# SamsungLabs/Metis

Hardware: NVIDIA H100
Metric: candidate plans evaluated/sec (higher is better)
Workload: dtype f64

## Files before the change

### metis_b200/csrc/metis_coop.cuh

```cuda
#pragma once

#include "metis_eval.cuh"

namespace metis {

struct CoopMail {
    int m;
    int err;
    int flag;
    int aux;
    double val;
    double val2;
    int k;
    int s_top;
    int top_skip;
    int pad2;
};

struct OneLane {
    bool reverse = false;
    MB_HD int lane() const { return 0; }
    MB_HD int width() const { return 1; }
    MB_HD bool leader() const { return true; }
    MB_HD void sync() const {}
    MB_HD bool any(bool p) const { return p; }
    MB_HD unsigned ballot(bool p) const { return p ? 1u : 0u; }
    MB_HD unsigned match_any(int) const { return 1u; }
    MB_HD int first_ge_window(const double *P, int n, int i0, int lo, double t) const {
        for (int k = 0; k < 32 && i0 + k <= n; ++k)
            if (P[i0 + k] >= t) return (k > 0 || i0 <= lo) ? i0 + k : -1;
        return -1;
    }
    MB_HD int first_ge(const double *P, int n, double t) const {
        int lo = 0, hi = n + 1;
        while (lo < hi) { const int mid = (lo + hi) >> 1; if (P[mid] >= t) hi = mid; else lo = mid + 1; }
        return lo;
    }
    MB_HD int bcast_last(int v) const { return v; }
    MB_HD static void assume_shared(const void *) {}
    MB_HD void argmax_first(double &, int &) const {}
    MB_HD void argmin_first(double &, int &) const {}
    MB_HD void imax_first(int &, int &) const {}
    MB_HD void imin_first(int &, int &) const {}
    MB_HD double max_all(double v) const { return v; }
    MB_HD int incl_scan(int v) const { return v; }
    MB_HD int last_lane(int v) const { return v; }
    MB_HD void mark(int) const {}
    MB_HD void note(int) const {}
    MB_HD void gate(int, int) const {}
};

enum CoopGate { kGateRun = 0, kGateBackward = 1, kGateLeftover = 2, kGateVote = 3, kGateAdjust = 4, kGateMemory = 5,
                kGateCost = 6 };

template <class X>
MB_HD int par_index(const X &, int i, int n) { (void)n; return i; }
MB_HD int par_index(const OneLane &x, int i, int n) { return x.reverse ? n - 1 - i : i; }

#define METIS_PAR(x, var, n) \
    for (int var##_i = (x).lane(), var = par_index((x), var##_i, (n)); var##_i < (n); \
         var##_i += (x).width(), var = par_index((x), var##_i, (n)))

struct FillState {
    int k;
    int s_top;
    bool top_skip;
};

template <int MAXS, int MAXL>
MB_HD_NOINLINE FillState seq_forward(const Tables &T, int S, Scratch<MAXS, MAXL> &w) {
    const int L = T.p.num_layers;
    const double *dlay = T.dlay;
    const int N = kH * L;
    const int lim = (N - 1 - kH) > 0 ? (N - 1 - kH) : 0;
    const int last = S - 1;
    FillState st{0, -1, false};
    if (S > 1) {
        int s = 0, j = 0;
        double c = w.capa[0];
        bool done = false;
#pragma unroll 1
        for (int r = 0; r + 1 < L && !done; ++r) {
            const double d = dlay[r];
            const int nsub = (r == L - 2) ? kH - 1 : kH;
            if (nsub == kH && c > 9.0 * d) {
                c -= d; c -= d; c -= d; c -= d; c -= d; c -= d; c -= d;
                j += kH;
                continue;
            }
#pragma unroll
            for (int q = 0; q < kH; ++q) {
                if (q < nsub && !done) {
                    if (c > d) {
                        c -= d;
                    } else {
                        w.capa[s] = c;
                        w.fe[s] = (uint16_t)((j + q) | kBroke);
                        ++s;
                        if (s >= last) done = true;
                        else c = w.capa[s];
                    }
                }
            }
            j += nsub;
        }
        if (s < last) {
            w.capa[s] = c;
            w.fe[s] = (uint16_t)lim;
#pragma unroll 1
            for (int t = s + 1; t < last; ++t) w.fe[t] = (uint16_t)lim;
            st.k = lim;
            st.s_top = s;
        } else {
            st.k = (w.fe[last - 1] & kPos) + 1;
            st.s_top = last - 1;
            st.top_skip = true;
        }
    }
    return st;
}

template <int MAXS, int MAXL>
MB_HD_NOINLINE int seq_backward(const Tables &T, int S, Scratch<MAXS, MAXL> &w, int k) {
    const int L = T.p.num_layers;
    const double *dlay = T.dlay;
    const int N = kH * L;
    const int last = S - 1;
    double c = w.capa[last];
    int r = L - 1;
    double d = dlay[r];
#pragma unroll 1
    for (int i = 0; i < kH; ++i) c -= d;
    int m = N - kH;
    bool full = false;
#pragma unroll 1
    while (m > k && !full) {
        --r;
        d = dlay[r];
        const int floor_j = kH * r > k ? kH * r : k;
#pragma unroll 1
        while (m > floor_j) {
            if (!(c > d)) { full = true; break; }
            c -= d;
            --m;
        }
    }
    if (!full) {
        int sp = S - 2;
#pragma unroll 1
        while (m > 0) {
            const int j = m - 1;
#pragma unroll 1
            while (sp >= 0 && (!(w.fe[sp] & kBroke) || (int)(w.fe[sp] & kPos) > j)) --sp;
            if (!(sp >= 0 && (int)(w.fe[sp] & kPos) == j)) break;
            const double dj = dlay[j / kH];
            if (!(c > dj)) break;
            c -= dj;
            m = j;
            w.fe[sp] |= kTaken;
        }
    }
    w.capa[last] = c;
    return m;
}

template <int MAXS, int MAXL>
MB_HD_NOINLINE int seq_skipped(const Tables &T, int S, Scratch<MAXS, MAXL> &w) {
    const double *dlay = T.dlay;
    const int last = S - 1;
    int start = 0;
#pragma unroll 1
    for (int s = 0; s < last; ++s) {
        const uint16_t e = w.fe[s];
        const int pos = e & kPos;
        const int next_start = pos + ((e & kBroke) ? 1 : 0);
        if ((e & (kBroke | kTaken)) != kBroke) { start = next_start; continue; }
        const int j = pos;
        int lo = 0;
        if (pos > start) {
            lo = s;
        } else {
#pragma unroll 1
            for (int u = s;; --u) {
                if (u < s) {
                    const int t = w.lstk[u];
                    const bool above = (t == last) || (fwd_nonempty(w, t) && fwd_start(w, t) > j);
                    if (!above) { lo = t; break; }
                }
                if (fwd_nonempty(w, u)) { lo = u; break; }
                if (u == 0) break;
            }
        }
        int hi = s + 1;
        if (hi < last && !((int)(w.fe[hi] & kPos) > next_start && !w.got[hi])) {
            ++hi;
#pragma unroll 1
            while (hi < last && (!fwd_nonempty(w, hi) || w.got[hi])) ++hi;
        }
        if (lo > hi) return METIS_FATAL_SCRATCH;
        int pick = lo;
        double best = w.capa[lo];
#pragma unroll 1
        for (int t = lo + 1; t <= hi; ++t)
            if (w.capa[t] > best) { best = w.capa[t]; pick = t; }
        w.capa[pick] -= dlay[j / kH];
        w.lstk[s] = (uint8_t)pick;
        w.got[pick] = 1;
        start = next_start;
    }
    return METIS_FATAL_NONE;
}

template <int MAXS, int MAXL>
MB_HD int middle_lo(int S, const Scratch<MAXS, MAXL> &w, const FillState &st) {
    const int last = S - 1;
    if (st.s_top < 0) return 0;
#pragma unroll 1
    for (int u = st.s_top;; --u) {
        if (u < st.s_top || st.top_skip) {
            const uint16_t eu = w.fe[u];
            if ((eu & (kBroke | kTaken)) == kBroke) {
                const int t2 = w.lstk[u];
                if (t2 != last) return t2;
            }
        }
        if (fwd_nonempty(w, u)) return u;
        if (u == 0) break;
    }
    return 0;
}

MB_HD_NOINLINE double seq_py_sum(const double *v, int n) {
    if (n <= 0) return 0.0;
    double f = 0.0 + v[0], c = 0.0;
#pragma unroll 4
    for (int i = 1; i < n; ++i) {
        const double x = v[i];
        const double t = f + x;
        if (fabs(f) >= fabs(x)) c += (f - t) + x;
        else c += (x - t) + f;
        f = t;
    }
    if (c != 0.0 && isfinite(c)) f += c;
    return f;
}

template <int MAXS, int MAXL, class X, bool ONE = false>
struct CoopEvaluator : PlanEvaluator<MAXS, MAXL, SerialUniform, ONE> {
    using Base = PlanEvaluator<MAXS, MAXL, SerialUniform, ONE>;
    using Base::T; using Base::w; using Base::pd; using Base::bs_total; using Base::nbad; using Base::aux;
    X x;
    CoopMail &mail;

    MB_HD CoopEvaluator(const Tables &t, Scratch<MAXS, MAXL> &s, CoopMail &mb, const X &lanes)
        : Base(t, s), x(lanes), mail(mb) {}

    MB_HD void shared_scratch() const { X::assume_shared(&w); X::assume_shared(&mail); }

    MB_HD void begin_coop(const PlanDesc &plan) {
        shared_scratch();
        pd = plan;
        bs_total = T.p.gbs / pd.batches;
        int lb = 0;
#pragma unroll 1
        while ((2 << lb) <= bs_total) ++lb;
        nbad = 0;
        x.sync();
        int carry = 0;
#pragma unroll 1
        for (int base = 0; base < pd.S; base += x.width()) {
            const int s = base + x.lane();
            const int g = s < pd.S ? pd.row[s] : 0;
            const int sz = s < pd.S ? (1 << g) : 0;
            const int inc = x.incl_scan(sz);
            if (s < pd.S) {
                w.gcode[s] = (uint8_t)g;
                w.tpc[s] = (uint8_t)(g > lb ? g - lb : 0);
                w.rs[s] = (uint16_t)(carry + inc - sz);
            }
            carry += x.last_lane(inc);
        }
        if (x.leader()) w.rs[pd.S] = (uint16_t)carry;
        x.sync();
    }

    MB_HD bool next_strategy_coop(bool have_state) {
        shared_scratch();
        int pick = 0x7FFFFFFF;
        if (have_state) {
            double best = INFINITY;
            bool none = true;
            METIS_PAR(x, s, pd.S) {
                if (w.gcode[s] != w.tpc[s] && (none || w.mstate[s] < best || (w.mstate[s] == best && s < pick))) {
                    pick = s; best = w.mstate[s]; none = false;
                }
            }
            x.argmin_first(best, pick);
        } else {
            int best = -1;
            METIS_PAR(x, s, pd.S) {
                const int ldp = (int)w.gcode[s] - (int)w.tpc[s];
                if (ldp != 0 && (ldp > best || (ldp == best && s < pick))) { pick = s; best = ldp; }
            }
            x.imax_first(best, pick);
        }
        if (pick == 0x7FFFFFFF) return false;
        const int g = w.gcode[pick], t = w.tpc[pick];
        nbad += (this->stage_bad(g, t + 1) ? 1 : 0) - (this->stage_bad(g, t) ? 1 : 0);
        x.sync();
        if (x.leader()) w.tpc[pick] = (uint8_t)(t + 1);
        x.sync();
        return true;
    }

    MB_HD_NOINLINE int first_error(const double *box, int n) {
        shared_scratch();
        x.sync();
        if (x.leader()) {
            mail.err = 0;
#pragma unroll 1
            for (int s = 0; s < n; ++s)
                if (box[s] != 0.0) {
                    uint32_t a;
                    mail.err = decode_error(box[s], a);
                    mail.aux = (int)a;
                    break;
                }
        }
        x.sync();
        aux = (uint32_t)mail.aux;
        return mail.err;
    }

    MB_HD int compute_performance_coop() {
        shared_scratch();
        bool failed = false;
        x.sync();
        METIS_PAR(x, s, pd.S) {
            double p;
            const int rc = this->stage_performance(s, p);
            w.perf[s] = p;
            w.extra[s] = encode_error(rc, aux);
            failed = failed || rc != 0;
        }
        if (x.any(failed)) return first_error(w.extra, pd.S);
        x.sync();
        if (x.leader()) mail.val = seq_py_sum(w.perf, pd.S);
        x.sync();
        const double tot = mail.val;
        if (tot == 0.0) return METIS_FATAL_ZERODIV;
        METIS_PAR(x, s, pd.S) w.perf[s] = w.perf[s] / tot;
        x.sync();
        return 0;
    }

    MB_HD bool forward_coop() {
        shared_scratch();
        const int S = pd.S, last = S - 1;
        const int L = T.p.num_layers;
        if (S < 4 || T.p.norm_len < L) { x.note(kPathSeqForward); return false; }
        const int N = kH * L;
        const int lim = (N - 1 - kH) > 0 ? (N - 1 - kH) : 0;
        const double *dsub = T.dsub;
        const double *P = T.psub;
        int a = 0, first_open = -1;
        int span = lim / last;
#pragma unroll 1
        for (int s = 0; s < last; ++s) {
            int b = lim;
            bool closed = false;
            if (a < lim) {
                const double t = w.perf[s] + P[a];
                int i0 = a + span - 14;
                if (i0 < a + 1) i0 = a + 1;
                int i = x.first_ge_window(P, N, i0, a + 1, t);
                if (i < 0) { x.note(kPathFirstGe); i = x.first_ge(P, N, t); }
                b = i - 1 > a ? i - 1 : a;
                if (b >= lim) b = lim; else closed = true;
                span = b - a;
            }
            if (x.leader()) { w.first[s] = (uint16_t)a; w.fe[s] = (uint16_t)(b | (closed ? kBroke : 0)); }
            if (!closed && first_open < 0) first_open = s;
            a = closed ? b + 1 : lim;
        }
        x.sync();
        x.mark(19);
        bool bad = false;
        METIS_PAR(x, s, last) {
            const int st = w.first[s];
            const uint16_t e = w.fe[s];
            const int b = e & kPos;
            double c = w.perf[s];
            bool fits = true;
#pragma unroll 4
            for (int j = st; j < b; ++j) {
                const double d = dsub[j];
                fits &= c > d;
                c -= d;
            }
            if (!fits || ((e & kBroke) && c > dsub[b])) bad = true;
            w.capa[s] = c;
        }
        if (x.any(bad)) {
            x.note(kPathVerifyFailed);
            x.sync();
            METIS_PAR(x, s, last) w.capa[s] = w.perf[s];
            return false;
        }
        if (x.leader()) {
            if (first_open < 0) { mail.k = a; mail.s_top = last - 1; mail.top_skip = 1; }
            else { mail.k = lim; mail.s_top = first_open; mail.top_skip = 0; }
        }
        return true;
    }

    MB_HD int fill_coop() {
        shared_scratch();
        const int S = pd.S, last = S - 1;
        const double *dlay = T.dlay;
        x.sync();
        const bool fwd = forward_coop();
        x.sync();
        x.gate(kGateBackward, 11);
        if (x.leader()) {
            if (!fwd) {
                x.mark(18);
                const FillState st = seq_forward<MAXS, MAXL>(T, S, w);
                mail.k = st.k; mail.s_top = st.s_top; mail.top_skip = st.top_skip ? 1 : 0;
                x.mark(11);
            }
            mail.m = seq_backward<MAXS, MAXL>(T, S, w, mail.k);
            mail.err = 0;
        }
        x.sync();
        x.gate(kGateLeftover, 12);
        const FillState st{mail.k, mail.s_top, mail.top_skip != 0};
        const int m = mail.m;
        if (st.s_top >= 0 && !st.top_skip) x.note(kPathTail);
        const int reach = st.s_top;
        bool irregular = false;
        METIS_PAR(x, s, reach + 1) {
            const int start = s == 0 ? 0 : (int)(w.fe[s - 1] & kPos) + ((w.fe[s - 1] & kBroke) ? 1 : 0);
            if (!((int)(w.fe[s] & kPos) > start)) irregular = true;
        }
        irregular = x.any(irregular);
        if (irregular) {
            x.note(kPathIrregular);
            if (x.leader()) mail.err = seq_skipped<MAXS, MAXL>(T, S, w);
            x.sync();
            if (mail.err) return mail.err;
        } else if (reach >= 0) {
            int carry = 0;
#pragma unroll 1
            for (int base = 0; base <= last; base += x.width()) {
                const int s = base + x.lane();
                bool has = false, o0 = false, o1 = false, has_prev = false;
                double c = 0.0, d = 0.0, d_prev = 0.0;
                int pos = 0;
                if (s <= last) {
                    c = w.capa[s];
                    if (s > 0 && s - 1 < last) {
                        const uint16_t ep = w.fe[s - 1];
                        has_prev = (ep & (kBroke | kTaken)) == kBroke;
                        if (has_prev) d_prev = dlay[(ep & kPos) / kH];
                    }
                    if (s < last) {
                        const uint16_t e = w.fe[s];
                        has = (e & (kBroke | kTaken)) == kBroke;
                        if (has) {
                            pos = e & kPos;
                            d = dlay[pos / kH];
                            const double cn = w.capa[s + 1];
                            o0 = cn > c;
                            o1 = has_prev ? cn > (c - d_prev) : o0;
                        }
                    }
                }
                const unsigned kmask = x.ballot(o0 == o1), vmask = x.ballot(o0);
                const unsigned below_me = x.lane() ? (0xFFFFFFFFu >> (32 - x.lane())) : 0u;
                const unsigned kin = kmask & below_me;
                const bool in = kin ? ((vmask >> (31 - clz32(kin))) & 1u) != 0u : carry != 0;
                const bool up = (o0 == o1) ? o0 : in;
                carry = x.bcast_last(up ? 1 : 0);
                x.sync();
                if (s <= last) {
                    double cc = c;
                    const bool got_prev = has_prev && in;
                    if (got_prev) cc -= d_prev;
                    if (has && !up) cc -= d;
                    if (got_prev || (has && !up)) w.capa[s] = cc;
                    if (has) w.lstk[s] = (uint8_t)(up ? s + 1 : s);
                }
            }
            x.sync();
        }
        x.mark(17);
        if (m > st.k) {
            x.note(kPathMiddle);
            if (x.leader()) mail.flag = middle_lo<MAXS, MAXL>(S, w, st);
            x.sync();
            int lo = mail.flag;
#pragma unroll 1
            for (int j = st.k; j < m; ++j) {
                int pick = 0x7FFFFFFF;
                double best = -INFINITY;
#pragma unroll 1
                for (int t = lo + x.lane(); t <= last; t += x.width())
                    if (w.capa[t] > best || (w.capa[t] == best && t < pick)) { best = w.capa[t]; pick = t; }
                x.argmax_first(best, pick);
                x.sync();
                if (x.leader()) {
                    w.capa[pick] = best - dlay[j / kH];
                    reinterpret_cast<uint8_t *>(w.subw)[j - st.k] = (uint8_t)pick;
                }
                x.sync();
                if (pick != last) lo = pick;
            }
        }
        return METIS_FATAL_NONE;
    }

    MB_HD int balance_coop() {
        shared_scratch();
        const int S = pd.S;
        const int L = T.p.num_layers;
        if (T.p.norm_len < L) return METIS_FATAL_INDEX;
        const double *lc = T.norm_lc;
        const int last = S - 1;
        x.sync();
        METIS_PAR(x, s, S) { w.capa[s] = w.perf[s]; w.got[s] = 0; }
        x.sync();
        x.mark(10);
        const int rc_tail = fill_coop();
        if (rc_tail) return rc_tail;
        const int m = mail.m;
        x.gate(kGateVote, 13);
        const int kfwd = mail.k;
        const int B = (L + 31) >> 5;
        METIS_PAR(x, blk, 32) {
            const int r0 = blk * B, r1 = r0 + B < L ? r0 + B : L;
            const int j0 = kH * r0;
            int t = 0;
            if (j0 < kfwd && j0 < m) {
                int lo = 0, hi = last - 1;
#pragma unroll 1
                while (lo < hi) {
                    const int mid = (lo + hi) >> 1;
                    const uint16_t e = w.fe[mid];
                    if ((int)(e & kPos) + ((e & kBroke) ? 1 : 0) <= j0) lo = mid + 1; else hi = mid;
                }
                t = lo;
            }
            uint16_t e = w.fe[t];
            int nxt = (int)(e & kPos) + ((e & kBroke) ? 1 : 0);
#pragma unroll 1
            for (int r = r0; r < r1; ++r) {
                int own = last;
                if (kH * r < m) {
                    uint64_t v = 0xFF00000000000000ULL;
#pragma unroll 1
                    for (int q = 0; q < kH; ++q) {
                        const int j = kH * r + q;
                        int st;
                        if (j >= m) st = last;
                        else if (j >= kfwd) st = reinterpret_cast<const uint8_t *>(w.subw)[j - kfwd];
                        else {
#pragma unroll 1
                            while (nxt <= j) { ++t; e = w.fe[t]; nxt = (int)(e & kPos) + ((e & kBroke) ? 1 : 0); }
                            st = t;
                            if (nxt - 1 == j && (e & kBroke)) st = (e & kTaken) ? last : (int)w.lstk[t];
                        }
                        v |= (uint64_t)st << (8 * q);
                    }
                    own = layer_owner(v, (T.p.corrected & METIS_FIX_Q5) != 0);
                }
                reinterpret_cast<uint8_t *>(w.ownerw)[r] = (uint8_t)own;
            }
        }
        METIS_PAR(x, s, S) w.cnt[s] = 0;
        x.sync();
        x.mark(14);
#pragma unroll 1
        for (int base = 0; base < L; base += x.width()) {
            const int r = base + x.lane();
            const int own = r < L ? (int)reinterpret_cast<const uint8_t *>(w.ownerw)[r] : (int)kDropped;
            const unsigned peers = x.match_any(own);
            if (own != (int)kDropped && x.lane() == ctz32(peers)) {
                const int n = popc32(peers), lo_r = r, hi_r = base + 31 - clz32(peers);
                const int have = w.cnt[own];
                if (have == 0 || lo_r < (int)w.first[own]) w.first[own] = (uint16_t)lo_r;
                if (have == 0 || hi_r > (int)w.lastl[own]) w.lastl[own] = (uint16_t)hi_r;
                w.cnt[own] = (uint16_t)(have + n);
            }
            x.sync();
        }
        METIS_PAR(x, s, S) {
            const int n = w.cnt[s];
            w.capa[s] = n ? w.perf[s] - range_sum<SerialUniform>(T, kRangeNorm, 0, lc, w.first[s], (int)w.lastl[s] + 1) : w.perf[s];
        }
        x.sync();
        x.gate(kGateAdjust, 15);
        uint8_t *owner = reinterpret_cast<uint8_t *>(w.ownerw);
#pragma unroll 1
        for (int n = 1; n <= 3; ++n) {
            int top = 0x7FFFFFFF;
            double maxc = -INFINITY;
            METIS_PAR(x, t, S)
                if (w.capa[t] > maxc || (w.capa[t] == maxc && t < top)) { maxc = w.capa[t]; top = t; }
            x.argmax_first(maxc, top);
            if (top == 0x7FFFFFFF) top = 0;
            int nb = -1;
            double val = INFINITY;
            if (top - 1 >= 0 && w.capa[top - 1] < val) { nb = top - 1; val = w.capa[top - 1]; }
            if (top + 1 < S && w.capa[top + 1] < val) { nb = top + 1; }
            if (nb < 0 || w.cnt[nb] <= 1) break;
            const int layer = (top > nb) ? w.lastl[nb] : w.first[nb];
            const double dl = lc[layer];
            const double ntop = w.capa[top] - dl;
            const double nnb = w.capa[nb] + dl;
            double newmax = -INFINITY;
            METIS_PAR(x, t, S) {
                const double v = (t == top) ? ntop : (t == nb) ? nnb : w.capa[t];
                if (v > newmax) newmax = v;
            }
            newmax = x.max_all(newmax);
            if (newmax > maxc) break;
            x.sync();
            if (x.leader()) {
                owner[layer] = (uint8_t)top;
                w.capa[top] = ntop;
                w.capa[nb] = nnb;
                if (top > nb) { int r = layer - 1; while (owner[r] != nb) --r; w.lastl[nb] = (uint16_t)r; }
                else          { int r = layer + 1; while (owner[r] != nb) ++r; w.first[nb] = (uint16_t)r; }
                if (w.cnt[top] == 0) { w.first[top] = (uint16_t)layer; w.lastl[top] = (uint16_t)layer; }
                else {
                    if (layer < (int)w.first[top]) w.first[top] = (uint16_t)layer;
                    if (layer > (int)w.lastl[top]) w.lastl[top] = (uint16_t)layer;
                }
                ++w.cnt[top];
                --w.cnt[nb];
            }
            x.sync();
        }
        x.mark(16);
        int carry = 0;
#pragma unroll 1
        for (int base = 0; base < S; base += x.width()) {
            const int s = base + x.lane();
            const int v = s < S ? (int)w.cnt[s] : 0;
            const int inc = x.incl_scan(v);
            if (s < S) w.part[s + 1] = (uint16_t)(carry + inc);
            carry += x.last_lane(inc);
        }
        if (x.leader()) w.part[0] = 0;
        x.sync();
        return METIS_FATAL_NONE;
    }

    MB_HD int adjust_performance_coop() {
        shared_scratch();
        const int S = pd.S;
        double *ratio = reinterpret_cast<double *>(w.subw);
        x.sync();
        METIS_PAR(x, s, S) {
            double av, adj, extra;
            this->stage_adjust(s, av, adj, extra);
            w.capa[s] = av;
            w.mstate[s] = adj;
            ratio[s] = extra;
        }
        x.sync();
        if (x.leader()) {
            double need = 0.;
#pragma unroll 4
            for (int s = 0; s < S; ++s) need += ratio[s];
            mail.val = need;
            mail.flag = seq_py_sum(w.capa, S) < need ? 1 : 0;
        }
        x.sync();
        if (mail.flag) return 1;
        METIS_PAR(x, s, S) w.extra[s] = 0.;
        x.sync();
        if (x.leader()) {
            double need = mail.val;
            int guard = 0;
            mail.err = 0;
// ... 181 lines not shown
```

### metis_b200/csrc/metis_eval.cuh

```cuda
#pragma once

#include <stdint.h>
#include <string.h>
#include <math.h>

#include "../../include/metis_b200.h"

#if defined(__CUDACC__)
#define MB_HD __host__ __device__ __forceinline__
#define MB_HD_NOINLINE __host__ __device__ __noinline__ inline
#else
#define MB_HD inline
#define MB_HD_NOINLINE inline
#endif

namespace metis {

constexpr int kH = 7;
constexpr double kMemCoef = 5.0;
constexpr uint8_t kDropped = 0xFF;

struct Tables {
    MetisProblem p;
    const int16_t *key_index;
    const double *lc;
    const double *mem;
    const double *exec_full;
    const double *fb_sync;
    const double *norm_lc;
    const double *type_memory, *bw_first, *bw_min;
    const uint8_t *run_type;
    const int32_t *run_end;
    const int32_t *q10_end;
    const double *dlay;
    const double *inv_exec;
    const double *ratio;
    const double *dpk;
    const double *pp_hidden;
    const double *pp_vocab;
    const double *psub;
    const double *dsub;
    const double *rsum;
};

constexpr int kDpk = 16;

struct DerivedLayout {
    int dlay, inv_exec, ratio, dpk, pp_hidden, pp_vocab, psub, dsub, total;
};

MB_HD DerivedLayout derived_layout(const MetisProblem &p) {
    DerivedLayout d;
    int o = 0;
    d.dlay = o; o += p.norm_len;
    d.inv_exec = o; o += p.num_keys;
    d.ratio = o; o += p.num_layers + 1;
    d.dpk = o; o += kDpk;
    d.pp_hidden = o; o += p.num_bs + 1;
    d.pp_vocab = o; o += (p.num_bs + 1) * p.num_tp;
    d.psub = o; o += (p.norm_len >= p.num_layers) ? kH * p.num_layers + 1 : 0;
    d.dsub = o; o += (p.norm_len >= p.num_layers) ? kH * p.num_layers : 0;
    d.total = o;
    return d;
}

MB_HD double derive_entry(const MetisProblem &p, const DerivedLayout &d, const double *norm_lc,
                          const double *exec_full, const double *bw_first, int i) {
    if (i < d.inv_exec) return norm_lc[i - d.dlay] / 7.0;
    if (i < d.ratio) return 1. / exec_full[i - d.inv_exec];
    if (i < d.dpk) return (double)(i - d.ratio) / (double)p.num_layers;
    const double bw = bw_first[0] * 1048576.0;
    if (i < d.pp_hidden) {
        const int dp = 1 << (i - d.dpk);
        return (double)(2 * (dp - 1)) / ((double)dp * bw);
    }
    if (i < d.pp_vocab) return (double)((int64_t)(i - d.pp_hidden) * p.sequence_length * p.hidden_size) / bw;
    if (i >= d.dsub) return norm_lc[(i - d.dsub) / kH] / 7.0;
    if (i >= d.psub) {
        const int j = i - d.psub, r = j / kH;
        double acc = 0.0;
        for (int t = 0; t < r; ++t) acc += norm_lc[t];
        return r < p.norm_len ? acc + norm_lc[r] * ((double)(j - r * kH) / 7.0) : acc;
    }
    const int e = i - d.pp_vocab;
    const int mbs = e / p.num_tp, tpc = e - mbs * p.num_tp;
    return ((double)((int64_t)mbs * p.sequence_length * p.vocab_size) / (double)(1 << tpc)) / bw;
}

MB_HD void bind_derived(Tables &T, const double *base) {
    const DerivedLayout d = derived_layout(T.p);
    T.dlay = base + d.dlay;
    T.inv_exec = base + d.inv_exec;
    T.ratio = base + d.ratio;
    T.dpk = base + d.dpk;
    T.pp_hidden = base + d.pp_hidden;
    T.pp_vocab = base + d.pp_vocab;
    T.psub = base + d.psub;
    T.dsub = base + d.dsub;
}

struct PlanDesc {
    uint32_t ordinal;
    int ns;
    int S;
    int label;
    int batches;
    const uint8_t *row;
    uint64_t geo;
};

MB_HD uint64_t pack_geo(int64_t row_offset, int S, int label, int ns, int div) {
    return (uint64_t)(row_offset & 0xFFFFFFFFLL) | ((uint64_t)((S - 1) & 0xFF) << 32) | ((uint64_t)((label - 1) & 0xFF) << 40) |
           ((uint64_t)(ns & 0xFF) << 48) | ((uint64_t)(div & 0xFF) << 56);
}

enum BalancerPath {
    kPathVerifyFailed = 0,
    kPathSeqForward = 1,
    kPathIrregular = 2,
    kPathMiddle = 3,
    kPathFirstGe = 4,
    kPathTail = 5,
    kPathVoteEnds = 6,
};

struct Serial {
    static constexpr bool kUniform = false;
    MB_HD void mark(int) const {}
    MB_HD void note(int) const {}
    MB_HD void converge() const {}
    MB_HD void rejoin(bool) {}
};
#if defined(__CUDACC__) && defined(METIS_PROFILE_PHASES)
constexpr int kBulkBatches = 31;
__device__ long long g_bulk_acc[32];
__shared__ long long s_bulk_t[32];
__shared__ int s_bulk_cur[32];
__device__ __forceinline__ void bulk_mark(unsigned group, int id) {
    __syncwarp(group);
    if ((int)(threadIdx.x & 31) == __ffs((int)group) - 1) {
        const int wi = threadIdx.x >> 5;
        const long long now = clock64();
        if (id == 1) atomicAdd((unsigned long long *)&g_bulk_acc[kBulkBatches], 1ULL);
        else atomicAdd((unsigned long long *)&g_bulk_acc[s_bulk_cur[wi] & 31], (unsigned long long)(now - s_bulk_t[wi]));
        s_bulk_cur[wi] = id;
        s_bulk_t[wi] = now;
    }
    __syncwarp(group);
}
#endif
#if defined(__CUDACC__)
struct Lockstep : Serial {
    unsigned mask;
    __device__ Lockstep() : mask(0xFFFFFFFFu) {}
    __device__ void converge() const { __syncwarp(mask); }
    __device__ void rejoin(bool p) { mask = __ballot_sync(0xFFFFFFFFu, p); }
#if defined(METIS_PROFILE_PHASES)
    __device__ void mark(int id) const { bulk_mark(__activemask(), id); }
#endif
};
#endif
struct SerialUniform : Serial {
    static constexpr bool kUniform = true;
};

constexpr uint64_t kOnes = 0x0101010101010101ULL;

constexpr uint16_t kBroke = 0x8000;
constexpr uint16_t kTaken = 0x4000;
constexpr uint16_t kPos = 0x3FFF;

template <int MAXS, int MAXL>
struct Scratch {
    double perf[MAXS];
    double capa[MAXS];
    double mstate[MAXS];
    double extra[MAXS];
    uint16_t fe[MAXS];
    uint16_t first[MAXS], lastl[MAXS], cnt[MAXS];
    uint16_t part[MAXS + 1];
    uint16_t rs[MAXS + 1];
    uint8_t gcode[MAXS];
    uint8_t tpc[MAXS];
    uint8_t lstk[MAXS];
    uint8_t got[MAXS];
    uint64_t ownerw[MAXL / 8 + 1];
    uint64_t subw[MAXL];
    static_assert(MAXL >= MAXS, "after the vote, subw holds one double per stage (CoopEvaluator's adjust and cost)");
};

MB_HD double py_sum_range(const double *x, int a, int b) {
    if (a >= b) return 0.0;
    double f = 0.0 + x[a];
    double c = 0.0;
    for (int i = a + 1; i < b; ++i) {
        const double v = x[i];
        const double t = f + v;
        if (fabs(f) >= fabs(v)) c += (f - t) + v;
        else c += (v - t) + f;
        f = t;
    }
    if (c != 0.0 && isfinite(c)) f += c;
    return f;
}

MB_HD_NOINLINE double py_sum_range_compact(const double *x, int a, int b) {
    if (a >= b) return 0.0;
    double f = 0.0 + x[a];
    double c = 0.0;
#pragma unroll 1
    for (int i = a + 1; i < b; ++i) {
        const double v = x[i];
        const double t = f + v;
        if (fabs(f) >= fabs(v)) c += (f - t) + v;
        else c += (v - t) + f;
        f = t;
    }
    if (c != 0.0 && isfinite(c)) f += c;
    return f;
}

template <class X>
MB_HD double sum_range(const double *x, int a, int b) {
    if constexpr (X::kUniform) return py_sum_range_compact(x, a, b);
    else return py_sum_range(x, a, b);
}

MB_HD void fill_range_sums(const double *row, int L, int a, double *out) {
    const int n = L + 1;
    double f = 0.0 + row[a];
    double c = 0.0;
    out[(size_t)(a + 1) * n + a] = f;
#if defined(__CUDA_ARCH__)
#pragma unroll 1
#endif
    for (int i = a + 1; i < L; ++i) {
        const double v = row[i];
        const double t = f + v;
        if (fabs(f) >= fabs(v)) c += (f - t) + v;
        else c += (v - t) + f;
        f = t;
        out[(size_t)(i + 1) * n + a] = (c != 0.0 && isfinite(c)) ? f + c : f;
    }
}
MB_HD int range_sum_tables(const MetisProblem &p) { return 2 * p.num_keys + 1; }
MB_HD const double *range_sum_row(const MetisProblem &p, int t, const double *mem, const double *lc, const double *norm) {
    if (t < p.num_keys) return mem + (size_t)t * p.lpad;
    if (t < 2 * p.num_keys) return lc + (size_t)(t - p.num_keys) * p.lpad;
    return p.norm_len >= p.num_layers ? norm : nullptr;
}

enum RangeTable { kRangeMem = 0, kRangeLc = 1, kRangeNorm = 2 };
template <class X>
MB_HD double range_sum(const Tables &T, int family, int key, const double *row, int a, int b) {
    if (a >= b) return 0.0;
    if (T.rsum && b <= T.p.num_layers) {
        const int n = T.p.num_layers + 1;
        const int t = family == kRangeMem ? key : family == kRangeLc ? T.p.num_keys + key : 2 * T.p.num_keys;
#if defined(__CUDA_ARCH__)
        return __ldg(&T.rsum[((size_t)t * n + b) * n + a]);
#else
        return T.rsum[((size_t)t * n + b) * n + a];
#endif
    }
    return sum_range<X>(row, a, b);
}

struct PySum {
    double f, c;
    int n;
    MB_HD PySum() : f(0.0), c(0.0), n(0) {}
    MB_HD void add(double v) {
        if (n == 0) { f = 0.0 + v; }
        else {
            const double t = f + v;
            if (fabs(f) >= fabs(v)) c += (f - t) + v;
            else c += (v - t) + f;
            f = t;
        }
        ++n;
    }
    MB_HD double result() const {
        double r = f;
        if (c != 0.0 && isfinite(c)) r += c;
        return r;
    }
};

MB_HD double pow2_neg(int k) {
    const uint64_t bits = (uint64_t)(1023 - k) << 52;
    double d;
    memcpy(&d, &bits, sizeof(d));
    return d;
}

MB_HD int type_of_rank(const Tables &T, int ns, int rank) {
    const int nt = T.p.num_types;
    const int32_t *end = T.run_end + ns * nt;
    const uint8_t *typ = T.run_type + ns * nt;
#pragma unroll 1
    for (int k = 0; k < nt; ++k)
        if (rank < end[k]) return typ[k];
    return typ[nt - 1];
}

MB_HD int type_of_q10(const Tables &T, int ns, int idx) {
    const int nt = T.p.num_types;
    const int32_t *end = T.q10_end + ns * nt;
    const uint8_t *typ = T.run_type + ns * nt;
#pragma unroll 1
    for (int k = 0; k < nt; ++k)
        if (idx < end[k]) return typ[k];
    return typ[nt - 1];
}

MB_HD int key_of(const Tables &T, int type, int tpc, int bs) {
    if (tpc >= T.p.num_tp || bs < 1 || bs > T.p.num_bs) return -1;
    return T.key_index[(type * T.p.num_tp + tpc) * T.p.num_bs + (bs - 1)];
}

template <int MAXS, int MAXL>
MB_HD int fwd_start(const Scratch<MAXS, MAXL> &w, int s) {
    if (s == 0) return 0;
    const uint16_t e = w.fe[s - 1];
    return (e & kPos) + ((e & kBroke) ? 1 : 0);
}

template <int MAXS, int MAXL>
MB_HD bool fwd_nonempty(const Scratch<MAXS, MAXL> &w, int s) {
    return (int)(w.fe[s] & kPos) > fwd_start(w, s);
}

MB_HD int popc64(uint64_t v) {
#if defined(__CUDA_ARCH__)
    return __popcll(v);
#else
    return __builtin_popcountll(v);
#endif
}
MB_HD int ctz64(uint64_t v) {
#if defined(__CUDA_ARCH__)
    return __ffsll((long long)v) - 1;
#else
    return __builtin_ctzll(v);
#endif
}
MB_HD int popc32(uint32_t v) {
#if defined(__CUDA_ARCH__)
    return __popc(v);
#else
    return __builtin_popcount(v);
#endif
}
MB_HD int ctz32(uint32_t v) {
#if defined(__CUDA_ARCH__)
    return __ffs((int)v) - 1;
#else
    return __builtin_ctz(v);
#endif
}
MB_HD int clz32(uint32_t v) {
#if defined(__CUDA_ARCH__)
    return __clz((int)v);
#else
    return __builtin_clz(v);
#endif
}
MB_HD int clz64(uint64_t v) {
#if defined(__CUDA_ARCH__)
    return __clzll((long long)v);
#else
    return __builtin_clzll(v);
#endif
}

MB_HD uint64_t swar_eq(uint64_t x, int c) {
    const uint64_t y = x ^ ((uint64_t)c * kOnes);
    const uint64_t lo7 = 0x7F7F7F7F7F7F7F7FULL;
    return ~((((y & lo7) + lo7) | y) | lo7);
}

MB_HD int swar_count(uint64_t x, int c) { return popc64(swar_eq(x, c) & 0x0080808080808080ULL); }

MB_HD int layer_owner(uint64_t v, bool plurality) {
    if (plurality) {
        int best = 0, own = (int)kDropped;
#pragma unroll 1
        for (int q = 0; q < kH; ++q) {
            const int cq = (int)((v >> (8 * q)) & 0xFF);
            const int n = swar_count(v, cq);
            if (n > best || (n == best && cq < own)) { best = n; own = cq; }
        }
        return own;
    }
    const int c3 = (int)((v >> 24) & 0xFF);
    if (swar_count(v, c3) * 2 > kH) return c3;
    const int c0 = (int)(v & 0xFF), c1 = (int)((v >> 8) & 0xFF), c2 = (int)((v >> 16) & 0xFF);
    if (swar_count(v, c0) * 2 > kH) return c0;
    if (c1 != c0 && swar_count(v, c1) * 2 > kH) return c1;
    if (c2 != c1 && c2 != c0 && swar_count(v, c2) * 2 > kH) return c2;
    return (int)kDropped;
// ... 1070 lines not shown
```

Baseline: 209.6 million.

## Add bucketed prefix-sum index to replace windowed search in forward stage split

Precomputes a uniform bucket index over the psub prefix-sum table, packed as uint16 entries into doubles in the derived table area. The forward stage-boundary loop then maps each target value to a bucket and takes a direct candidate, checking only neighbours, instead of running a windowed first-greater-or-equal search per stage. It falls back to the old search when the bucket guess misses and to the old loop when the index scale is invalid. The derived table grows, and the fill rule for open stages changes, which could affect correctness in edge cases.

Result: faster. 216.7 million, median of 6 (+3.4%).

```diff
diff --git a/metis_b200/csrc/metis_coop.cuh b/metis_b200/csrc/metis_coop.cuh
--- a/metis_b200/csrc/metis_coop.cuh
+++ b/metis_b200/csrc/metis_coop.cuh
@@ -245,6 +245,41 @@
     return f;
 }
 
+template <class X>
+MB_HD_NOINLINE int psub_search(const X &x, const double *P, int N, int i0, int lo, double t) {
+    int i = x.first_ge_window(P, N, i0, lo, t);
+    if (i < 0) {
+        x.note(kPathFirstGe);
+        i = x.first_ge(P, N, t);
+        if (i < lo) i = lo;
+    }
+    return i;
+}
+
+MB_HD unsigned bucket_of(double u) {
+#ifdef __CUDA_ARCH__
+    return __double2uint_rz(u);
+#else
+    return u > 0.0 ? (unsigned)u : 0u;
+#endif
+}
+
+template <class X>
+MB_HD int psub_lookup(const X &x, const double *P, const uint16_t *IX, double scale, int N, int lo, double t, double &p) {
+    int i = IX[bucket_of(t * scale)];
+    if (i < lo) i = lo;
+    const double *q = P + i;
+    const double pm = q[-1], p0 = q[0], p1 = q[1];
+    if ((pm < t || i == lo) && p1 >= t) {
+        const bool up = !(p0 >= t);
+        p = up ? p1 : p0;
+        return up ? i + 1 : i;
+    }
+    i = psub_search(x, P, N, i, lo, t);
+    p = P[i];
+    return i;
+}
+
 template <int MAXS, int MAXL, class X, bool ONE = false>
 struct CoopEvaluator : PlanEvaluator<MAXS, MAXL, SerialUniform, ONE> {
     using Base = PlanEvaluator<MAXS, MAXL, SerialUniform, ONE>;
@@ -364,24 +399,48 @@
         const double *dsub = T.dsub;
         const double *P = T.psub;
         int a = 0, first_open = -1;
-        int span = lim / last;
-#pragma unroll 1
-        for (int s = 0; s < last; ++s) {
-            int b = lim;
-            bool closed = false;
-            if (a < lim) {
-                const double t = w.perf[s] + P[a];
-                int i0 = a + span - 14;
-                if (i0 < a + 1) i0 = a + 1;
-                int i = x.first_ge_window(P, N, i0, a + 1, t);
-                if (i < 0) { x.note(kPathFirstGe); i = x.first_ge(P, N, t); }
-                b = i - 1 > a ? i - 1 : a;
-                if (b >= lim) b = lim; else closed = true;
-                span = b - a;
-            }
-            if (x.leader()) { w.first[s] = (uint16_t)a; w.fe[s] = (uint16_t)(b | (closed ? kBroke : 0)); }
-            if (!closed && first_open < 0) first_open = s;
-            a = closed ? b + 1 : lim;
+        const double scale = T.pidx[0];
+        if (scale > 0.0) {
+            const uint16_t *IX = reinterpret_cast<const uint16_t *>(T.pidx + 1);
+            const double plim = P[lim];
+            double pa = P[0];
+            int s = 0;
+#pragma unroll 1
+            for (; s < last; ++s) {
+                const double t = w.perf[s] + pa;
+                if (!(a < lim && t <= plim)) break;
+                const int i = psub_lookup(x, P, IX, scale, N, a + 1, t, pa);
+                if (x.leader()) { w.first[s] = (uint16_t)a; w.fe[s] = (uint16_t)((i - 1) | kBroke); }
+                a = i;
+            }
+            if (s < last) {
+                first_open = s;
+                if (x.leader()) {
+#pragma unroll 1
+                    for (int u = s; u < last; ++u) { w.first[u] = (uint16_t)(u == s ? a : lim); w.fe[u] = (uint16_t)lim; }
+                }
+                a = lim;
+            }
+        } else {
+            int span = lim / last;
+#pragma unroll 1
+            for (int s = 0; s < last; ++s) {
+                int b = lim;
+                bool closed = false;
+                if (a < lim) {
+                    const double t = w.perf[s] + P[a];
+                    int i0 = a + span - 14;
+                    if (i0 < a + 1) i0 = a + 1;
+                    int i = x.first_ge_window(P, N, i0, a + 1, t);
+                    if (i < 0) { x.note(kPathFirstGe); i = x.first_ge(P, N, t); }
+                    b = i - 1 > a ? i - 1 : a;
+                    if (b >= lim) b = lim; else closed = true;
+                    span = b - a;
+                }
+                if (x.leader()) { w.first[s] = (uint16_t)a; w.fe[s] = (uint16_t)(b | (closed ? kBroke : 0)); }
+                if (!closed && first_open < 0) first_open = s;
+                a = closed ? b + 1 : lim;
+            }
         }
         x.sync();
         x.mark(19);
diff --git a/metis_b200/csrc/metis_eval.cuh b/metis_b200/csrc/metis_eval.cuh
--- a/metis_b200/csrc/metis_eval.cuh
+++ b/metis_b200/csrc/metis_eval.cuh
@@ -40,13 +40,14 @@
     const double *pp_vocab;
     const double *psub;
     const double *dsub;
+    const double *pidx;
     const double *rsum;
 };
 
 constexpr int kDpk = 16;
 
 struct DerivedLayout {
-    int dlay, inv_exec, ratio, dpk, pp_hidden, pp_vocab, psub, dsub, total;
+    int dlay, inv_exec, ratio, dpk, pp_hidden, pp_vocab, psub, dsub, pidx, total;
 };
 
 MB_HD DerivedLayout derived_layout(const MetisProblem &p) {
@@ -60,8 +61,50 @@
     d.pp_vocab = o; o += (p.num_bs + 1) * p.num_tp;
     d.psub = o; o += (p.norm_len >= p.num_layers) ? kH * p.num_layers + 1 : 0;
     d.dsub = o; o += (p.norm_len >= p.num_layers) ? kH * p.num_layers : 0;
+    d.pidx = o; o += (p.norm_len >= p.num_layers) ? 1 + (kH * p.num_layers + 1 + 3) / 4 : 0;
     d.total = o;
     return d;
+}
+
+MB_HD double psub_at(double acc, double lc_r, int q) { return acc + lc_r * ((double)q / 7.0); }
+
+MB_HD double psub_index_entry(const MetisProblem &p, const double *norm_lc, int k) {
+    const int L = p.num_layers, N = kH * L;
+    const int lim = (N - 1 - kH) > 0 ? (N - 1 - kH) : 0;
+    bool ok = N > 0;
+    double acc = 0.0;
+    for (int r = 0; r < L; ++r) {
+        ok = ok && norm_lc[r] >= 0.0 && norm_lc[r] <= 1.7976931348623157e308;
+        acc += norm_lc[r];
+    }
+    const double top = L < p.norm_len ? psub_at(acc, norm_lc[L], 0) : acc;
+    const double scale = ok && top > 0.0 && top <= 1.7976931348623157e308 ? (double)N / top : 0.0;
+    if (!(scale > 0.0 && scale <= 1.7976931348623157e308)) return 0.0;
+    if (k == 0) return scale;
+    double f[kH];
+    for (int q = 0; q < kH; ++q) f[q] = (double)q / 7.0;
+    uint64_t bits = 0;
+    int r = 0;
+    acc = 0.0;
+    for (int e = 0; e < 4; ++e) {
+        const double g = (double)(4 * (k - 1) + e);
+        int ix = lim;
+        while (kH * r < lim) {
+            const double nxt = acc + norm_lc[r];
+            if (nxt * scale >= g) {
+                int q = 0;
+                while (q < kH && !((acc + norm_lc[r] * f[q]) * scale >= g)) ++q;
+                ix = kH * r + q < lim ? kH * r + q : lim;
+                break;
+            }
+            acc = nxt;
+            ++r;
+        }
+        bits |= (uint64_t)ix << (16 * e);
+    }
+    double v;
+    memcpy(&v, &bits, sizeof(v));
+    return v;
 }
 
 MB_HD double derive_entry(const MetisProblem &p, const DerivedLayout &d, const double *norm_lc,
@@ -75,12 +118,13 @@
         return (double)(2 * (dp - 1)) / ((double)dp * bw);
     }
     if (i < d.pp_vocab) return (double)((int64_t)(i - d.pp_hidden) * p.sequence_length * p.hidden_size) / bw;
+    if (i >= d.pidx) return psub_index_entry(p, norm_lc, i - d.pidx);
     if (i >= d.dsub) return norm_lc[(i - d.dsub) / kH] / 7.0;
     if (i >= d.psub) {
         const int j = i - d.psub, r = j / kH;
         double acc = 0.0;
         for (int t = 0; t < r; ++t) acc += norm_lc[t];
-        return r < p.norm_len ? acc + norm_lc[r] * ((double)(j - r * kH) / 7.0) : acc;
+        return r < p.norm_len ? psub_at(acc, norm_lc[r], j - r * kH) : acc;
     }
     const int e = i - d.pp_vocab;
     const int mbs = e / p.num_tp, tpc = e - mbs * p.num_tp;
@@ -97,6 +141,7 @@
     T.pp_vocab = base + d.pp_vocab;
     T.psub = base + d.psub;
     T.dsub = base + d.dsub;
+    T.pidx = base + d.pidx;
 }
 
 struct PlanDesc {
```
